# ketanfatania/QMRI-PnP-Recon-POC

Measured on NVIDIA B200. Metric: ADMM slice-iterations/s (224x224x10 slices; step = 120-slice PnP-ADMM recon + T1/T2/PD matching), higher is better.
Workload: dtype f32 (x-update fp32 FFT; denoiser split-bf16 tcgen05, fp32 accumulate; matching fp32)

## Files before the change

qmri-pnp-recon-poc_b200/csrc/conv_tc.cu:

```cuda
#include <cuda.h>
#include <cuda_bf16.h>
#include <math.h>
#include <stdlib.h>
#include <string.h>
#include <time.h>
#include <unistd.h>

#include "common.cuh"
#include "conv_kernels.h"

namespace {

constexpr int TC_THREADS = 192;
constexpr int PAIR_THREADS = 224;
constexpr int TC_BM = 128;
constexpr int TC_BK = 64;
constexpr uint32_t A_TILE_BYTES = TC_BM * TC_BK * 2;

template <int BN>
struct TcCfg {
    static constexpr uint32_t B_TILE_BYTES = BN * TC_BK * 2;
    static constexpr uint32_t STAGE_BYTES = 2 * A_TILE_BYTES + 2 * B_TILE_BYTES;
    static constexpr int STAGES = (BN == 64) ? 4 : 3;
    static constexpr uint32_t TMEM_COLS = 2 * BN;
// ... 76 lines not shown
        "elect.sync _|e, 0xffffffff;\n\t"
        "setp.ne.b32 p, %4, 0;\n\t"
        "@e tcgen05.mma.cta_group::1.kind::f16 [%0], %1, %2, %3, p;\n\t}"
        ::"r"(tmem_d), "l"(desc_a), "l"(desc_b), "r"(idesc), "r"(accumulate)
        : "memory");
}
__device__ __forceinline__ void tc_commit_elect(uint64_t* bar) {
    asm volatile(
        "{\n\t.reg .pred e;\n\t"
        "elect.sync _|e, 0xffffffff;\n\t"
        "@e tcgen05.commit.cta_group::1.mbarrier::arrive::one.shared::cluster.b64 [%0];\n\t}"
        ::"r"(smem_u32(bar))
        : "memory");
}

__device__ __forceinline__ uint64_t umma_desc(uint32_t saddr) {
    const uint64_t lo = (uint64_t)((saddr >> 4) & 0x3FFF) | ((uint64_t)1 << 16);
    const uint64_t hi = (uint64_t)64 | ((uint64_t)1 << 14) | ((uint64_t)2 << 29);
    return lo | (hi << 32);
}

__device__ __forceinline__ uint32_t pack_bf16(float a, float b) {
    __nv_bfloat162 t = __floats2bfloat162_rn(a, b);
    return *reinterpret_cast<uint32_t*>(&t);
}
__device__ __forceinline__ void unpack_bf16(uint32_t u, float& a, float& b) {
    a = __uint_as_float(u << 16);
    b = __uint_as_float(u & 0xffff0000u);
}


struct TcMaps {
    CUtensorMap a_hi[4], a_lo[4];
// ... 439 lines not shown
        __syncwarp();
        cluster_sync_all();
        if (warp >= 2) tc_epilogue_reduce_dsmem<BN>(p, reinterpret_cast<const float*>(smem), cs_row, (int)cluster_ctarank(), cs_o, cs_ok);
        __syncwarp();
        cluster_sync_all();
    }
    tc_fence_before();
    __syncthreads();
    if (warp == 1) {
        tc_fence_after();
        asm volatile("tcgen05.dealloc.cta_group::1.sync.aligned.b32 %0, %1;" ::"r"(tmem_base), "r"(Cfg::TMEM_COLS));
    }
}


template <int NA, int STACK>
struct PairCfg {
    static constexpr int NOUT = STACK ? NA / 2 : NA;
    static constexpr uint32_t A_PLANE = 20480;
    static constexpr uint32_t A_SLOT = 2 * A_PLANE;
    static constexpr uint32_t B1_BYTES = (NA / 2) * 128;
    static constexpr uint32_t B2_BYTES = STACK ? (NA / 4) * 128 : B1_BYTES;
    static constexpr uint32_t B_STAGE = B1_BYTES + B2_BYTES;
    static constexpr int AS = (NA == 128) ? 3 : 2;
    static constexpr int ASB = 4;
    static constexpr int BS = (NA == 128) ? 8 : (STACK ? 5 : 4);
    static constexpr bool DUAL_OK = STACK && NA == 128;
    static constexpr int EPW = DUAL_OK ? 8 : 4;
    static constexpr int THREADS = DUAL_OK ? 352 : PAIR_THREADS;
    static constexpr uint32_t TMEM_COLS = DUAL_OK ? 512 : 2 * NA;
    static constexpr uint32_t RESW_BYTES = 9 * B1_BYTES;
    static constexpr size_t STAGE_AREA = (size_t)AS * A_SLOT + (size_t)BS * B_STAGE;
    static constexpr size_t SMEM = STAGE_AREA + 1024 + 256;
};

__device__ __forceinline__ uint32_t mapa_rank(uint32_t saddr, uint32_t rank) {
    uint32_t r;
    asm volatile("mapa.shared::cluster.u32 %0, %1, %2;" : "=r"(r) : "r"(saddr), "r"(rank));
    return r;
}
__device__ __forceinline__ void mbar_arrive_cluster(uint32_t cluster_addr) {
    asm volatile("mbarrier.arrive.release.cluster.shared::cluster.b64 _, [%0];" ::"r"(cluster_addr) : "memory");
}
__device__ __forceinline__ void mbar_arrive_cluster_relaxed(uint32_t cluster_addr) {
    asm volatile("mbarrier.arrive.relaxed.cluster.shared::cluster.b64 _, [%0];" ::"r"(cluster_addr) : "memory");
}
__device__ __forceinline__ void tma2_load_4d(void* dst, const CUtensorMap* tm, uint32_t bar_cluster_addr, int c0, int c1, int c2, int c3) {
    asm volatile(
        "cp.async.bulk.tensor.4d.cta_group::2.shared::cluster.global.tile.mbarrier::complete_tx::bytes [%0], [%1, {%3, %4, %5, %6}], [%2];"
        ::"r"(smem_u32(dst)), "l"(tm), "r"(bar_cluster_addr), "r"(c0), "r"(c1), "r"(c2), "r"(c3)
        : "memory");
}
__device__ __forceinline__ void tma2_load_2d(void* dst, const CUtensorMap* tm, uint32_t bar_cluster_addr, int c0, int c1) {
    asm volatile(
        "cp.async.bulk.tensor.2d.cta_group::2.shared::cluster.global.tile.mbarrier::complete_tx::bytes [%0], [%1, {%3, %4}], [%2];"
        ::"r"(smem_u32(dst)), "l"(tm), "r"(bar_cluster_addr), "r"(c0), "r"(c1)
        : "memory");
}
__device__ __forceinline__ void tma_prefetch_l2_4d(const CUtensorMap* tm, int c0, int c1, int c2, int c3) {
    asm volatile("cp.async.bulk.prefetch.tensor.4d.L2.global.tile [%0, {%1, %2, %3, %4}];" ::"l"(tm), "r"(c0), "r"(c1), "r"(c2), "r"(c3) : "memory");
}
__device__ __forceinline__ void tc2_commit(uint64_t* bar) {
    asm volatile("tcgen05.commit.cta_group::2.mbarrier::arrive::one.shared::cluster.multicast::cluster.b64 [%0], %1;" ::"r"(smem_u32(bar)), "h"((uint16_t)3)
                 : "memory");
}
__device__ __forceinline__ void tc2_mma(uint32_t tmem_d, uint64_t desc_a, uint64_t desc_b, uint32_t idesc, uint32_t accumulate) {
    asm volatile(
        "{\n\t.reg .pred p;\n\t"
        "setp.ne.b32 p, %4, 0;\n\t"
        "tcgen05.mma.cta_group::2.kind::f16 [%0], %1, %2, %3, p;\n\t}"
        ::"r"(tmem_d), "l"(desc_a), "l"(desc_b), "r"(idesc), "r"(accumulate)
        : "memory");
}

__device__ __forceinline__ void tc2_mma_elect(uint32_t tmem_d, uint64_t desc_a, uint64_t desc_b, uint32_t idesc, uint32_t accumulate) {
    asm volatile(
        "{\n\t.reg .pred p, e;\n\t"
        "elect.sync _|e, 0xffffffff;\n\t"
        "setp.ne.b32 p, %4, 0;\n\t"
        "@e tcgen05.mma.cta_group::2.kind::f16 [%0], %1, %2, %3, p;\n\t}"
        ::"r"(tmem_d), "l"(desc_a), "l"(desc_b), "r"(idesc), "r"(accumulate)
        : "memory");
}
__device__ __forceinline__ void tc2_commit_elect(uint64_t* bar) {
    asm volatile(
        "{\n\t.reg .pred e;\n\t"
        "elect.sync _|e, 0xffffffff;\n\t"
        "@e tcgen05.commit.cta_group::2.mbarrier::arrive::one.shared::cluster.multicast::cluster.b64 [%0], %1;\n\t}"
        ::"r"(smem_u32(bar)), "h"((uint16_t)3)
        : "memory");
}

template <int NA, int STACK>
__device__ __forceinline__ void pair_acc16(uint32_t taddr, uint32_t taddr2, int c0, float* v, bool resw = false) {
    uint32_t a[16];
    tc_ld16(taddr + c0, a);
    if (STACK) {
        uint32_t b[16];
        tc_ld16(taddr + (resw ? (c0 < NA / 4 ? 3 * NA / 4 : NA / 4) : NA / 2) + c0, b);
        if (taddr2) {
            uint32_t c[16];
            tc_ld16(taddr2 + c0, c);
            tc_wait_ld();
#pragma unroll
            for (int j = 0; j < 16; ++j) v[j] = (__uint_as_float(a[j]) + __uint_as_float(c[j])) + __uint_as_float(b[j]);
        } else {
            tc_wait_ld();
#pragma unroll
            for (int j = 0; j < 16; ++j) v[j] = __uint_as_float(a[j]) + __uint_as_float(b[j]);
        }
    } else {
        tc_wait_ld();
#pragma unroll
        for (int j = 0; j < 16; ++j) v[j] = __uint_as_float(a[j]);
    }
}

template <int NA, int STACK>
__global__ void __launch_bounds__(PairCfg<NA, STACK>::THREADS, 1)
tc_conv3x3_pair_kernel(const __grid_constant__ CUtensorMap tmA_hi, const __grid_constant__ CUtensorMap tmA_lo,
                       const __grid_constant__ CUtensorMap tmB_hi, const __grid_constant__ CUtensorMap tmB_lo,
                       const __grid_constant__ CUtensorMap tmB_h2, const __grid_constant__ CUtensorMap tmB_l2,
                       const __grid_constant__ CUtensorMap tmO_hi, const __grid_constant__ CUtensorMap tmO_lo,
                       const __grid_constant__ CUtensorMap tmR_hi, const __grid_constant__ CUtensorMap tmR_lo, const TcK p) {
    using Cfg = PairCfg<NA, STACK>;
    constexpr int AS = Cfg::AS, BS = Cfg::BS, NOUT = Cfg::NOUT;
    extern __shared__ unsigned char tc_smem_raw[];
    const uint32_t raw = smem_u32(tc_smem_raw);
    unsigned char* smem = tc_smem_raw + ((1024u - (raw & 1023u)) & 1023u);
    unsigned char* smemB = smem + (size_t)AS * Cfg::A_SLOT;
    uint64_t* bars = reinterpret_cast<uint64_t*>(smemB + (size_t)BS * Cfg::B_STAGE);
    constexpr int ASB = Cfg::ASB;
    uint64_t* fullA = bars;
    uint64_t* emptyA = bars + ASB;
    uint64_t* fullB = bars + 2 * ASB;
    uint64_t* emptyB = bars + 2 * ASB + BS;
    uint64_t* tfull = bars + 2 * ASB + 2 * BS;
    uint64_t* tempty = tfull + 2;
    uint32_t* tmem_slot = reinterpret_cast<uint32_t*>(tempty + 2);

    const int warp = __shfl_sync(0xffffffffu, threadIdx.x >> 5, 0), lane = threadIdx.x & 31;
    const int cblocks = p.Cin / TC_BK;
    const int U = 3 * cblocks;
    const int NT = p.Cout / NOUT;
    const int tiles_xy = p.tiles_x * p.tiles_y;
    const int ptiles = tiles_xy * p.S;
    const int pgroups = (ptiles + 1) / 2;
    const int total_work = pgroups * NT * p.nsplit;
    const int crank = (int)cluster_ctarank();
    const int cidx = blockIdx.x >> 1, nclusters = gridDim.x >> 1;
    const uint32_t slab_bytes = (uint32_t)((p.BH + 2) * p.BW * 128);
    const uint32_t dy_bytes = (uint32_t)(p.BW * 128);
    const bool dual = Cfg::DUAL_OK && (p.dual & 1);
    const bool resw = Cfg::DUAL_OK && p.resw && p.Cin == TC_BK;
    const uint32_t a_stage = resw ? 2 * slab_bytes : Cfg::A_SLOT;
    const uint32_t a_plane = resw ? slab_bytes : Cfg::A_PLANE;
    const bool tma_out = resw && p.tma_out;
    const bool res_tma = tma_out && p.res_tma;
    constexpr uint32_t OUT_BYTES = 2 * TC_BM * 128;
    const int obufs = p.tma_out == 1 ? 1 : 2;
    const int as_fit = (int)((Cfg::STAGE_AREA - Cfg::RESW_BYTES - (tma_out ? obufs * OUT_BYTES : 0u)) / (2 * slab_bytes));
    uint64_t* fullR = fullB + 2;
    uint64_t* emptyR = fullB + 4;
    uint64_t* outFull = fullB + 6;
    const int as_cap = (p.resw >= 2 && p.resw < Cfg::ASB) ? p.resw : Cfg::ASB;
    const int AS_EFF = resw ? (as_fit < as_cap ? as_fit : as_cap) : AS;
    unsigned char* smemW = smem;
    unsigned char* smemO = smem + Cfg::RESW_BYTES;
    unsigned char* smemA = resw ? smem + Cfg::RESW_BYTES + (tma_out ? obufs * OUT_BYTES : 0u) : smem;

    if (threadIdx.x == 0) {
        const uint32_t nissue = dual ? 2u : 1u;
        for (int s = 0; s < ASB; ++s) {
            mbar_init(&fullA[s], 1);
            mbar_init(&emptyA[s], nissue);
        }
        for (int s = 0; s < BS; ++s) {
            mbar_init(&fullB[s], 1);
            mbar_init(&emptyB[s], nissue);
        }
        for (int a = 0; a < 2; ++a) {
            mbar_init(&tfull[a], nissue);
            mbar_init(&tempty[a], 2 * Cfg::EPW);
            if (tma_out) mbar_init(&outFull[a], Cfg::EPW);
        }
        asm volatile("fence.mbarrier_init.release.cluster;" ::: "memory");
        tma_prefetch_desc(&tmA_hi);
        tma_prefetch_desc(&tmA_lo);
        tma_prefetch_desc(&tmB_hi);
        tma_prefetch_desc(&tmB_lo);
        tma_prefetch_desc(&tmB_h2);
        tma_prefetch_desc(&tmB_l2);
        tma_prefetch_desc(&tmO_hi);
        tma_prefetch_desc(&tmO_lo);
        tma_prefetch_desc(&tmR_hi);
        tma_prefetch_desc(&tmR_lo);
    }
// ... 30 lines not shown
                const int r = w / p.nsplit;
                const int nt = r % NT;
                const int pt = (r / NT) * 2 + crank;
                const int txy = pt % tiles_xy;
                const int s = (pt < ptiles) ? pt / tiles_xy : p.S;
                const int x0 = (txy % p.tiles_x) * p.BW, y0 = (txy / p.tiles_x) * p.BH;
                const int u0 = (split * U) / p.nsplit, u1 = ((split + 1) * U) / p.nsplit;
                if (p.l2pf && w + nclusters < total_work) {
                    const int w2 = w + nclusters;
                    const int r2 = w2 / p.nsplit, split2 = w2 % p.nsplit;
                    const int pt2 = (r2 / NT) * 2 + crank;
                    if (pt2 < ptiles) {
                        const int txy2 = pt2 % tiles_xy, s2 = pt2 / tiles_xy;
                        const int px0 = (txy2 % p.tiles_x) * p.BW, py0 = (txy2 / p.tiles_x) * p.BH;
                        const int v0 = (split2 * U) / p.nsplit, v1 = ((split2 + 1) * U) / p.nsplit;
                        for (int u = v0; u < v1; ++u) {
                            const int cb = u / 3, dxi = u - 3 * cb;
                            tma_prefetch_l2_4d(&tmA_hi, cb * TC_BK, px0 + dxi - 1, py0 - 1, s2);
                            tma_prefetch_l2_4d(&tmA_lo, cb * TC_BK, px0 + dxi - 1, py0 - 1, s2);
                        }
                    }
                }
                for (int u = u0; u < u1; ++u) {
                    const int cb = u / 3, dxi = u - 3 * cb;
                    TC_TRACE(0, (w << 12) | (u << 4) | 1);
                    {
                        TC_PROF_T0();
                        mbar_wait(&emptyA[sa], pa ^ 1);
                        TC_PROF_ADD(prof_w5);
                    }
                    unsigned char* st = smemA + (size_t)sa * a_stage;
                    if (p.dual & 256) {
                        if (crank == 0) mbar_arrive(&fullA[sa]);
                    } else {
                    if (crank == 0) mbar_expect_tx(&fullA[sa], 4 * slab_bytes);
                    const uint32_t barA = mapa_rank(smem_u32(&fullA[sa]), 0);
                    tma2_load_4d(st, &tmA_hi, barA, cb * TC_BK, x0 + dxi - 1, y0 - 1, s);
                    tma2_load_4d(st + a_plane, &tmA_lo, barA, cb * TC_BK, x0 + dxi - 1, y0 - 1, s);
                    }
                    if (++sa == AS_EFF) {
                        sa = 0;
                        pa ^= 1;
                    }
                    for (int dyi = 0; dyi < 3 && !resw; ++dyi) {
                        const int kcol = (dyi * 3 + dxi) * p.Cin + cb * TC_BK;
                        TC_TRACE(0, (w << 12) | (u << 4) | (2 + dyi));
                        mbar_wait(&emptyB[sb], pb ^ 1);
                        unsigned char* sbp = smemB + (size_t)sb * Cfg::B_STAGE;
                        if (crank == 0) mbar_expect_tx(&fullB[sb], 2 * Cfg::B_STAGE);
                        const uint32_t barB = mapa_rank(smem_u32(&fullB[sb]), 0);
                        if (STACK) {
                            tma2_load_2d(sbp, crank == 0 ? &tmB_hi : &tmB_lo, barB, kcol, 0);
                            tma2_load_2d(sbp + Cfg::B1_BYTES, &tmB_h2, barB, kcol, crank * (NOUT / 2));
                        } else {
                            tma2_load_2d(sbp, &tmB_hi, barB, kcol, nt * NOUT + crank * (NA / 2));
                            tma2_load_2d(sbp + Cfg::B1_BYTES, &tmB_lo, barB, kcol, nt * NOUT + crank * (NA / 2));
                        }
// ... 25 lines not shown
            for (int w = cidx; w < total_work; w += nclusters, ++it) {
                const int split = w % p.nsplit;
                const int u0 = (split * U) / p.nsplit, u1 = ((split + 1) * U) / p.nsplit;
                const int ab = it & 1;
                const uint32_t aphase = (it >> 1) & 1;
                if (lane == 0) TC_TRACE(1, (w << 12) | 0xF00);
                {
                    TC_PROF_T0();
                    mbar_wait(&tempty[ab], aphase ^ 1);
                    TC_PROF_ADD(prof_w1);
                    ++prof_n;
                }
                tc_fence_after();
                const uint32_t tmem_d = tmem_base + (uint32_t)(ab * NA);
                for (int u = u0; u < u1; ++u) {
                    if (lane == 0) TC_TRACE(1, (w << 12) | (u << 4) | 1);
                    {
                        TC_PROF_T0();
                        mbar_wait(&fullA[sa], pa);
                        TC_PROF_ADD(prof_w0);
                    }
                    tc_fence_after();
                    const uint32_t ha = smem_u32(smemA + (size_t)sa * a_stage);
                    const long long issue_t0 = p.prof ? clock64() : 0;
                    for (int dyi = 0; dyi < 3; ++dyi) {
                        if (lane == 0) TC_TRACE(1, (w << 12) | (u << 4) | (2 + dyi));
                        if (!resw) {
                            mbar_wait(&fullB[sb], pb);
                            tc_fence_after();
                        }
                        if (p.dual & 16) continue;
                        const uint32_t sbase = resw ? smem_u32(smemW + (size_t)(dyi * 3 + (u - 3 * (u / 3))) * Cfg::B1_BYTES)
                                                    : smem_u32(smemB + (size_t)sb * Cfg::B_STAGE);
                        const uint64_t a_hi = umma_desc(ha + dyi * dy_bytes), a_lo = umma_desc(ha + a_plane + dyi * dy_bytes);
                        const uint64_t b_1 = umma_desc(sbase), b_2 = umma_desc(resw ? sbase : sbase + Cfg::B1_BYTES);
#pragma unroll
                        for (int k = 0; k < TC_BK / 16; ++k) {
                            const uint64_t ko = (uint64_t)(k * 2);
                            const uint32_t acc = ((u - u0) | dyi | k) ? 1u : 0u;
                            if (STACK) {
                                tc2_mma_elect(tmem_d, a_hi + ko, b_1 + ko, idesc_full, acc);
                                if (!dual) tc2_mma_elect(tmem_d, a_lo + ko, b_2 + ko, idesc_half, 1u);
                            } else {
                                tc2_mma_elect(tmem_d, a_hi + ko, b_1 + ko, idesc_full, acc);
                                tc2_mma_elect(tmem_d, a_hi + ko, b_2 + ko, idesc_full, 1u);
                                tc2_mma_elect(tmem_d, a_lo + ko, b_1 + ko, idesc_full, 1u);
                            }
                        }
                        if (!resw) {
                            tc2_commit_elect(&emptyB[sb]);
                            if (++sb == BS) {
                                sb = 0;
                                pb ^= 1;
                            }
                        }
                    }
                    if (p.prof) prof_w8 += (unsigned long long)(clock64() - issue_t0);
                    {
                        TC_PROF_T0();
                        tc2_commit_elect(&emptyA[sa]);
                        TC_PROF_ADD(prof_w9);
                    }
                    if (++sa == AS_EFF) {
                        sa = 0;
                        pa ^= 1;
                    }
                }
                {
                    TC_PROF_T0();
                    tc2_commit_elect(&tfull[ab]);
                    TC_PROF_ADD(prof_w9);
                }
            }
            if (lane == 0) {
            TC_PROF_PUT(8, prof_w8);
            TC_PROF_PUT(9, prof_w9);
            TC_PROF_PUT(2, clock64() - role_t0);
            }
            if (p.prof && lane == 0) {
                unsigned long long role_ns1;
// ... 25 lines not shown
                const int txy = pt % tiles_xy, s = pt / tiles_xy;
                const int sbuf = obufs == 2 ? (it & 1) : 0;
                mbar_wait(&outFull[sbuf], (uint32_t)(obufs == 2 ? it >> 1 : it) & 1u);
                if (pt < ptiles && !(p.dual & 32)) {
                    const int tx0 = (txy % p.tiles_x) * p.BW, ty0 = (txy / p.tiles_x) * p.BH;
                    tma_store_4d(&tmO_hi, smem_u32(smemO) + (uint32_t)sbuf * OUT_BYTES, 0, tx0, ty0, s);
                    tma_store_4d(&tmO_lo, smem_u32(smemO) + (uint32_t)sbuf * OUT_BYTES + TC_BM * 128u, 0, tx0, ty0, s);
                }
                asm volatile("cp.async.bulk.commit_group;" ::: "memory");
                asm volatile("cp.async.bulk.wait_group.read 0;" ::: "memory");
                if (res_tma) load_residual(w + obufs * nclusters, sbuf);
                else mbar_arrive(&emptyR[sbuf]);
            }
            asm volatile("cp.async.bulk.wait_group 0;" ::: "memory");
        }
        if (lane == 0 && crank == 0 && dual) {
            const uint32_t idesc_half = (1u << 4) | (1u << 7) | (1u << 10) | ((uint32_t)(256 >> 4) << 24) | ((uint32_t)((NA / 2) >> 3) << 17);
            int sa = 0, sb = 0;
            uint32_t pa = 0, pb = 0;
            int it = 0;
            for (int w = cidx; w < total_work; w += nclusters, ++it) {
                const int split = w % p.nsplit;
                const int u0 = (split * U) / p.nsplit, u1 = ((split + 1) * U) / p.nsplit;
                const int ab = it & 1;
                const uint32_t aphase = (it >> 1) & 1;
                if (resw && it == 0) {
                    mbar_wait(&fullB[0], 0);
                    tc_fence_after();
                }
                mbar_wait(&tempty[ab], aphase ^ 1);
                tc_fence_after();
                const uint32_t tmem_d2 = tmem_base + (uint32_t)(2 * NA + ab * (NA / 2));
                for (int u = u0; u < u1; ++u) {
                    mbar_wait(&fullA[sa], pa);
                    tc_fence_after();
                    const uint32_t ha = smem_u32(smemA + (size_t)sa * a_stage);
                    for (int dyi = 0; dyi < 3; ++dyi) {
                        if (!resw) {
                            mbar_wait(&fullB[sb], pb);
                            tc_fence_after();
                        }
                        const uint32_t sbase = resw ? smem_u32(smemW + (size_t)(dyi * 3 + (u - 3 * (u / 3))) * Cfg::B1_BYTES)
                                                    : smem_u32(smemB + (size_t)sb * Cfg::B_STAGE);
                        const uint64_t a_lo = umma_desc(ha + a_plane + dyi * dy_bytes);
                        const uint64_t b_2 = umma_desc(resw ? sbase : sbase + Cfg::B1_BYTES);
#pragma unroll
                        for (int k = 0; k < TC_BK / 16; ++k) {
                            const uint64_t ko = (uint64_t)(k * 2);
                            tc2_mma(tmem_d2, a_lo + ko, b_2 + ko, idesc_half, ((u - u0) | dyi | k) ? 1u : 0u);
                        }
                        if (!resw) {
                            tc2_commit(&emptyB[sb]);
                            if (++sb == BS) {
                                sb = 0;
                                pb ^= 1;
                            }
                        }
                    }
                    tc2_commit(&emptyA[sa]);
                    if (++sa == AS_EFF) {
                        sa = 0;
                        pa ^= 1;
                    }
                }
                tc2_commit(&tfull[ab]);
            }
        }
    } else {
        const int lg = warp & 3;
        const int row = lg * 32 + lane;
        int it = 0;
        const long long role_t0 = p.prof ? clock64() : 0;
        unsigned long long prof_w3 = 0, prof_w10 = 0, prof_w11 = 0, prof_w12 = 0, prof_w13 = 0;
        for (int w = cidx; w < total_work; w += nclusters, ++it) {
            const int split = w % p.nsplit;
            const int r = w / p.nsplit;
            const int ab = it & 1;
            const uint32_t aphase = (it >> 1) & 1;
            const int nt = r % NT;
            const int pt = (r / NT) * 2 + crank;
            const bool live = pt < ptiles;
            const int txy = pt % tiles_xy;
            const int s = pt / tiles_xy;
            const int x = (txy % p.tiles_x) * p.BW + row % p.BW;
            const int y = (txy / p.tiles_x) * p.BH + row / p.BW;
            const bool ok = live && (x < p.W) && (y < p.H);
            const size_t o = (((size_t)s * p.H + y) * p.W + x) * p.Cout + (size_t)nt * NOUT;
            const uint32_t taddr = tmem_base + ((uint32_t)(lg * 32) << 16) + (uint32_t)(ab * NA);
            const uint32_t taddr2 = dual ? tmem_base + ((uint32_t)(lg * 32) << 16) + (uint32_t)(2 * NA + ab * (NA / 2)) : 0u;
            const uint32_t tempty_leader = mapa_rank(smem_u32(&tempty[ab]), 0);
            if (lane == 0) TC_TRACE(2 + lg, (w << 12) | 1);
            if (p.nsplit == 1) {
                if constexpr (Cfg::DUAL_OK) {
                    const int sbuf = obufs == 2 ? (it & 1) : 0;
                    const uint32_t suse = (uint32_t)(obufs == 2 ? it >> 1 : it);
                    const uint32_t orow_hi = smem_u32(smemO) + (uint32_t)sbuf * OUT_BYTES + (uint32_t)row * 128u, orow_lo = orow_hi + TC_BM * 128u;
                    const int r7 = row & 7;
                    const bool g_r1 = ok && !res_tma && (p.res1_hi != nullptr), g_r2 = ok && (p.res2_hi != nullptr);
                    uint4 q2[4];
                    if (g_r2) {
                        const int c0 = (Cfg::EPW == 8 && warp >= 7) ? NOUT / 2 : 0;
                        q2[0] = *reinterpret_cast<const uint4*>(p.res2_hi + o + c0);
                        q2[1] = *reinterpret_cast<const uint4*>(p.res2_hi + o + c0 + 8);
                        q2[2] = *reinterpret_cast<const uint4*>(p.res2_lo + o + c0);
                        q2[3] = *reinterpret_cast<const uint4*>(p.res2_lo + o + c0 + 8);
                    }
                    if (tma_out) {
                        TC_PROF_T0();
                        if (res_tma) mbar_wait(&fullR[sbuf], suse & 1u);
                        else mbar_wait(&emptyR[sbuf], (suse & 1u) ^ 1u);
// ... 93 lines not shown
                            const uint4* gl = reinterpret_cast<const uint4*>(p.res2_lo + o + h0);
    #pragma unroll
                            for (int i = 0; i < PRE / 8; ++i) add_split8(rs + 8 * i, gh[i], gl[i]);
                        }
                        if (h0 == 0) {
                            TC_PROF_T0();
                            mbar_wait(&tfull[ab], aphase);
                            TC_PROF_ADD(prof_w3);
                            tc_fence_after();
                        }
                        if (p.dual & 32) continue;
    #pragma unroll
                        for (int c1 = 0; c1 < PRE; c1 += 16) {
                            const int cc = h0 + c1;
                            float v[16];
                            pair_acc16<NA, STACK>(taddr, taddr2, cc, v, resw);
                            if (has_r1 || has_r2) {
    #pragma unroll
                                for (int j = 0; j < 16; ++j) v[j] += rs[c1 + j];
                            }
                            if (ok) store_split16(p.out_hi + o + cc, p.out_lo + o + cc, v, p.relu);
                        }
                    }
                    tc_fence_before();
                    __syncwarp();
                    if (lane == 0) mbar_arrive_cluster(tempty_leader);
                }
            } else {
                mbar_wait(&tfull[ab], aphase);
                tc_fence_after();
                const int t = pt * NT + nt;
                float* prow0 = p.partial + ((size_t)t * p.nsplit * TC_BM + row) * NOUT;
                if (live) {
                    float* prow = prow0 + (size_t)split * TC_BM * NOUT;
#pragma unroll 1
                    for (int cc = 0; cc < NOUT; cc += 16) {
                        float v[16];
                        pair_acc16<NA, STACK>(taddr, taddr2, cc, v, resw);
                        float4* d = reinterpret_cast<float4*>(prow + cc);
#pragma unroll
                        for (int q = 0; q < 4; ++q) d[q] = make_float4(v[4 * q], v[4 * q + 1], v[4 * q + 2], v[4 * q + 3]);
                    }
                }
                tc_fence_before();
                __syncwarp();
                if (lane == 0) mbar_arrive_cluster(tempty_leader);
                if (live) {
                    __threadfence();
                    __syncwarp();
                    int old = 0;
                    if (lane == 0) old = atomicAdd(&p.tickets[t * 4 + lg], 1);
                    old = __shfl_sync(0xffffffffu, old, 0);
                    if (old == p.nsplit - 1) {
                        __threadfence();
                        if (lane == 0) p.tickets[t * 4 + lg] = 0;
                        if (ok) tc_epilogue_reduce<NOUT>(p, prow0, o);
                    }
                }
            }
        }
        if (threadIdx.x == 64) {
            TC_PROF_PUT(4, clock64() - role_t0);
            TC_PROF_PUT(3, prof_w3);
            TC_PROF_PUT(10, prof_w10);
            TC_PROF_PUT(11, prof_w11);
            TC_PROF_PUT(12, prof_w12);
            TC_PROF_PUT(13, prof_w13);
        }
    }
    if (lane == 0) TC_TRACE(6, 0x1000 + warp);
    tc_fence_before();
    __syncthreads();
    if (threadIdx.x == 0) TC_TRACE(7, 1);
    cluster_sync_all();
    if (warp == 1) {
        tc_fence_after();
        asm volatile("tcgen05.dealloc.cta_group::2.sync.aligned.b32 %0, %1;" ::"r"(tmem_base), "r"(Cfg::TMEM_COLS));
// ... 208 lines not shown
    k.tma_out = 0;
    k.res_tma = 0;
    k.l2pf = 0;
    k.prof = nullptr;
    if (BN == 64) {
        if (p.mode == TC_CONV3X3) return launch_tc<64, 0>(ctx, maps, k, grid);
        if (p.mode == TC_DOWN2X2) return launch_tc<64, 1>(ctx, maps, k, grid);
        return launch_tc<64, 2>(ctx, maps, k, grid);
    }
    if (p.mode == TC_CONV3X3) return launch_tc<128, 0>(ctx, maps, k, grid);
    if (p.mode == TC_DOWN2X2) return launch_tc<128, 1>(ctx, maps, k, grid);
    return launch_tc<128, 2>(ctx, maps, k, grid);
}

int tc_slab_tile_shape(int W, int H, int* BW, int* BH) {
    const int cand[2][2] = {{16, 8}, {8, 16}};
    int best = 0;
    double best_eff = -1;
    for (int i = 0; i < 2; ++i) {
        int bw = cand[i][0], bh = cand[i][1];
        double eff = ((double)W * H) / ((double)((W + bw - 1) / bw * bw) * ((H + bh - 1) / bh * bh));
        if (i == 1) eff *= 1.04;
        if (eff > best_eff + 1e-9) {
            best_eff = eff;
            best = i;
        }
    }
    *BW = cand[best][0];
    *BH = cand[best][1];
    return QMRI_OK;
}

void tc_pair_weight_boxes(int Cout, int* rows_main, int* rows_h2) {
    if (Cout >= 256) {
        *rows_main = 128;
        *rows_h2 = 128;
    } else {
        *rows_main = Cout;
        *rows_h2 = Cout / 2;
    }
}

template <int NA, int STACK>
static int launch_pair(qmri_ctx* ctx, const TcConvParams& p, TcK k) {
// ... 11 lines not shown
    const int U = 3 * (p.Cin / TC_BK);
    int nsplit = 1;
    if (p.partial && p.tickets && 2 * groups <= max_clusters) {
        nsplit = max_clusters / groups;
        if (nsplit > U / 2) nsplit = U / 2;
        if (nsplit > 8) nsplit = 8;
        if (nsplit < 1) nsplit = 1;
    }
    k.nsplit = nsplit;
    const int work = groups * nsplit;
    const int nclusters = work < max_clusters ? work : max_clusters;
    cudaLaunchConfig_t cfg = {};
    static const int dual_on = getenv("QMRI_TC_DUAL") ? atoi(getenv("QMRI_TC_DUAL")) : 0;
    static const bool resw_off = getenv("QMRI_TC_RESW") && !strcmp(getenv("QMRI_TC_RESW"), "0");
    static const int resw_stages = getenv("QMRI_TC_RESW") ? atoi(getenv("QMRI_TC_RESW")) : 1;
    k.dual = Cfg::DUAL_OK ? (dual_on & ~1) : 0;
    static const int dbg_layer = getenv("QMRI_TC_DBG_LAYER") ? atoi(getenv("QMRI_TC_DBG_LAYER")) : -1;
    static int launch_no = 0;
    bool dbg_this = true;
    if (Cfg::DUAL_OK && dbg_layer >= 0) {
        dbg_this = (launch_no++ % 16) == dbg_layer;
        if (!dbg_this) k.dual = 0;
    }
    k.resw = (Cfg::DUAL_OK && !resw_off && p.Cin == TC_BK) ? (resw_stages >= 2 ? resw_stages : 1) : 0;
    const char* tmaout_s = getenv("QMRI_TC_TMAOUT");
    const bool tma_out_off = tmaout_s && !strcmp(tmaout_s, "0");
    const char* outbuf_s = getenv("QMRI_TC_OUTBUF");
    const int outbuf_env = outbuf_s ? atoi(outbuf_s) : 0;
    k.tma_out = (k.resw && p.mapO_hi && p.mapO_lo && !tma_out_off) ? (outbuf_env == 1 || outbuf_env == 2 ? outbuf_env : (p.res1_hi ? 2 : 1)) : 0;
    k.res_tma = (k.tma_out && p.res1_hi && p.mapR_hi && p.mapR_lo) ? 1 : 0;
    static const int l2pf_env = getenv("QMRI_TC_L2PF") ? atoi(getenv("QMRI_TC_L2PF")) : 0;
    k.l2pf = l2pf_env > 0 ? 1 : 0;
    cfg.gridDim = dim3(nclusters * 2);
    cfg.blockDim = dim3(Cfg::THREADS);
    cfg.dynamicSmemBytes = Cfg::SMEM;
    cfg.stream = ctx->stream;
    cudaLaunchAttribute attr[2];
    attr[0].id = cudaLaunchAttributeClusterDimension;
    attr[0].val.clusterDim.x = 2;
    attr[0].val.clusterDim.y = 1;
    attr[0].val.clusterDim.z = 1;
    attr[1].id = cudaLaunchAttributeProgrammaticStreamSerialization;
    attr[1].val.programmaticStreamSerializationAllowed = tc_pdl_enabled() ? 1 : 0;
    cfg.attrs = attr;
// ... 298 lines not shown
    cfg.dynamicSmemBytes = SW_SMEM;
    cfg.stream = ctx->stream;
    cudaLaunchAttribute attr[1];
    attr[0].id = cudaLaunchAttributeProgrammaticStreamSerialization;
    attr[0].val.programmaticStreamSerializationAllowed = tc_pdl_enabled() ? 1 : 0;
    cfg.attrs = attr;
    cfg.numAttrs = 1;
    QCUDA(cudaLaunchKernelEx(&cfg, tc_conv64_swap_kernel, *(const CUtensorMap*)p.mapA_hi[0], *(const CUtensorMap*)p.mapA_lo[0], (const SwapK)k));
    QLAUNCH_CHECK(ctx);
    return QMRI_OK;
}

int conv3x3_tc_pair(qmri_ctx* ctx, const TcConvParams& p) {
    if (p.Cin % TC_BK) return qmri_fail(QMRI_EINVAL, "conv3x3_tc_pair: Cin %% 64");
    if (p.Cout != 64 && p.Cout != 128 && p.Cout % 256) return qmri_fail(QMRI_EINVAL, "conv3x3_tc_pair: Cout %d", p.Cout);
    if (p.BW % 8 || p.BW * p.BH != TC_BM || (p.BH + 2) * p.BW * 128 > (int)PairCfg<256, 0>::A_PLANE)
        return qmri_fail(QMRI_EINVAL, "conv3x3_tc_pair: tile %d x %d not supported", p.BW, p.BH);
    if (!p.mapA_hi[0] || !p.mapA_lo[0] || !p.mapB_hi || !p.mapB_lo || !p.mapB_h2) return qmri_fail(QMRI_EINVAL, "conv3x3_tc_pair: missing tensor map");
    TcK k;
    k.out_hi = p.out_hi; k.out_lo = p.out_lo;
    k.res1_hi = p.res1_hi; k.res1_lo = p.res1_lo;
    k.res2_hi = p.res2_hi; k.res2_lo = p.res2_lo;
    k.partial = p.partial; k.tickets = p.tickets;
    k.S = p.S; k.H = p.H; k.W = p.W; k.Cin = p.Cin; k.Cout = p.Cout;
    k.BW = p.BW; k.BH = p.BH; k.tiles_x = p.tiles_x; k.tiles_y = p.tiles_y;
    k.relu = p.relu; k.nsplit = 1; k.trace = nullptr; k.cluster_splitk = 0; k.dual = 0; k.resw = 0; k.tma_out = 0; k.res_tma = 0; k.l2pf = 0; k.prof = nullptr;
    if (p.Cout == 64) return launch_pair<128, 1>(ctx, p, k);
    if (p.Cout == 128) return launch_pair<256, 1>(ctx, p, k);
    return launch_pair<256, 0>(ctx, p, k);
}
```

qmri-pnp-recon-poc_b200/csrc/unetres.cu:

```cuda
#include <stdlib.h>
#include <string.h>

#include <vector>

#include "common.cuh"
#include "conv_kernels.h"
#include "unetres.h"

static const int NC[4] = {64, 128, 256, 512};

namespace {

struct LayerDesc {
    int kind;
    int cin, cout;
};

std::vector<LayerDesc> layer_table(int in_nc) {
    std::vector<LayerDesc> L;
    L.push_back({3, in_nc, NC[0]});
    for (int lvl = 0; lvl < 3; ++lvl) {
        for (int i = 0; i < 8; ++i) L.push_back({0, NC[lvl], NC[lvl]});
        L.push_back({1, NC[lvl], NC[lvl + 1]});
    }
// ... 295 lines not shown
    }
}

static int build_act_maps(qmri_net* net, int H, int W) {
    if (net->amap_ws == net->ws && net->amap_chunk == net->chunk && net->amap_H == H && net->amap_W == W) return QMRI_OK;
    uint16_t *hi[3][4], *lo[3][4];
    tc_buffers(net, H, W, hi, lo);
    for (int l = 0; l < 4; ++l) {
        int BW, BH;
        tc_tile_shape(W >> l, H >> l, &BW, &BH);
        for (int b = 0; b < 3; ++b) {
            QCHECK(tc_make_act_map(&net->amap[b][l][0], hi[b][l], net->chunk, H >> l, W >> l, NC[l], BW, BH));
            QCHECK(tc_make_act_map(&net->amap[b][l][1], lo[b][l], net->chunk, H >> l, W >> l, NC[l], BW, BH));
            int SW, SH;
            tc_slab_tile_shape(W >> l, H >> l, &SW, &SH);
            QCHECK(tc_make_act_map(&net->amap_slab[b][l][0], hi[b][l], net->chunk, H >> l, W >> l, NC[l], SW, SH + 2));
            QCHECK(tc_make_act_map(&net->amap_slab[b][l][1], lo[b][l], net->chunk, H >> l, W >> l, NC[l], SW, SH + 2));
            if (l == 0) {
                QCHECK(tc_make_act_map(&net->amap_tile[b][0], hi[b][0], net->chunk, H, W, NC[0], SW, SH));
                QCHECK(tc_make_act_map(&net->amap_tile[b][1], lo[b][0], net->chunk, H, W, NC[0], SW, SH));
            }
            if (l == 0 && conv64_swap_supported(W, H, NC[0], NC[0])) {
                QCHECK(tc_make_act_map(&net->amap_swap[b][0], hi[b][0], net->chunk, H, W, NC[0], 16, 16));
                QCHECK(tc_make_act_map(&net->amap_swap[b][1], lo[b][0], net->chunk, H, W, NC[0], 16, 16));
            }
            if (l < 3) {
                int DW, DH;
                tc_tile_shape(W >> (l + 1), H >> (l + 1), &DW, &DH);
                for (int tap = 0; tap < 4; ++tap) {
                    QCHECK(tc_make_down_map(&net->amap_down[b][l][tap][0], hi[b][l], net->chunk, H >> l, W >> l, NC[l], tap >> 1, tap & 1, DW, DH));
                    QCHECK(tc_make_down_map(&net->amap_down[b][l][tap][1], lo[b][l], net->chunk, H >> l, W >> l, NC[l], tap >> 1, tap & 1, DW, DH));
                }
// ... 241 lines not shown
```

Before: 1664.

## Load one halo slab per channel block and reuse it across dx taps

The pair conv kernel now TMA-loads a single (BW+2)x(BH+2) halo slab per 64-channel block, instead of three dx-shifted slabs. The MMA descriptors offset into it by dxi*128 bytes with a row stride of (BW+2)*128. This cuts A-operand TMA traffic and mbarrier round-trips per channel block roughly threefold, with the slab tile fixed at 8x16. The experimental dual-issue MMA path is removed, and the L2 prefetch is simplified to one prefetch per channel block. The fixed tile shape may pad worse for some layer sizes, and the non-default descriptor stride must match the swizzled layout.

```diff
diff --git a/qmri-pnp-recon-poc_b200/csrc/conv_tc.cu b/qmri-pnp-recon-poc_b200/csrc/conv_tc.cu
--- a/qmri-pnp-recon-poc_b200/csrc/conv_tc.cu
+++ b/qmri-pnp-recon-poc_b200/csrc/conv_tc.cu
@@ -114,9 +114,9 @@
         : "memory");
 }
 
-__device__ __forceinline__ uint64_t umma_desc(uint32_t saddr) {
+__device__ __forceinline__ uint64_t umma_desc(uint32_t saddr, uint32_t sbo = 1024) {
     const uint64_t lo = (uint64_t)((saddr >> 4) & 0x3FFF) | ((uint64_t)1 << 16);
-    const uint64_t hi = (uint64_t)64 | ((uint64_t)1 << 14) | ((uint64_t)2 << 29);
+    const uint64_t hi = (uint64_t)(sbo >> 4) | ((uint64_t)1 << 14) | ((uint64_t)2 << 29);
     return lo | (hi << 32);
 }
 
@@ -586,24 +586,30 @@
 }
 
 
+constexpr int PAIR_BW = 8, PAIR_BH = 16;
 template <int NA, int STACK>
 struct PairCfg {
     static constexpr int NOUT = STACK ? NA / 2 : NA;
-    static constexpr uint32_t A_PLANE = 20480;
+    static constexpr uint32_t SLAB_BYTES = (PAIR_BW + 2) * (PAIR_BH + 2) * 128;
+    static constexpr uint32_t A_PLANE = (SLAB_BYTES + 1023) & ~1023u;
     static constexpr uint32_t A_SLOT = 2 * A_PLANE;
     static constexpr uint32_t B1_BYTES = (NA / 2) * 128;
     static constexpr uint32_t B2_BYTES = STACK ? (NA / 4) * 128 : B1_BYTES;
     static constexpr uint32_t B_STAGE = B1_BYTES + B2_BYTES;
-    static constexpr int AS = (NA == 128) ? 3 : 2;
+    static constexpr int AS = 2;
     static constexpr int ASB = 4;
     static constexpr int BS = (NA == 128) ? 8 : (STACK ? 5 : 4);
-    static constexpr bool DUAL_OK = STACK && NA == 128;
-    static constexpr int EPW = DUAL_OK ? 8 : 4;
-    static constexpr int THREADS = DUAL_OK ? 352 : PAIR_THREADS;
-    static constexpr uint32_t TMEM_COLS = DUAL_OK ? 512 : 2 * NA;
+    static constexpr bool C64 = STACK && NA == 128;
+    static constexpr int EPW = C64 ? 8 : 4;
+    static constexpr int THREADS = C64 ? 352 : PAIR_THREADS;
+    static constexpr uint32_t TMEM_COLS = 2 * NA;
     static constexpr uint32_t RESW_BYTES = 9 * B1_BYTES;
-    static constexpr size_t STAGE_AREA = (size_t)AS * A_SLOT + (size_t)BS * B_STAGE;
+    static constexpr uint32_t OUT_BYTES = 2 * TC_BM * 128;
+    static constexpr size_t RESW_AREA = (size_t)RESW_BYTES + OUT_BYTES + 2 * (size_t)A_SLOT;
+    static constexpr size_t RING_AREA = (size_t)AS * A_SLOT + (size_t)BS * B_STAGE;
+    static constexpr size_t STAGE_AREA = (C64 && RESW_AREA > RING_AREA) ? RESW_AREA : RING_AREA;
     static constexpr size_t SMEM = STAGE_AREA + 1024 + 256;
+    static_assert(SMEM <= 227 * 1024, "pair kernel: dynamic shared memory over 227 KB");
 };
 
 __device__ __forceinline__ uint32_t mapa_rank(uint32_t saddr, uint32_t rank) {
@@ -631,18 +637,6 @@
 }
 __device__ __forceinline__ void tma_prefetch_l2_4d(const CUtensorMap* tm, int c0, int c1, int c2, int c3) {
     asm volatile("cp.async.bulk.prefetch.tensor.4d.L2.global.tile [%0, {%1, %2, %3, %4}];" ::"l"(tm), "r"(c0), "r"(c1), "r"(c2), "r"(c3) : "memory");
-}
-__device__ __forceinline__ void tc2_commit(uint64_t* bar) {
-    asm volatile("tcgen05.commit.cta_group::2.mbarrier::arrive::one.shared::cluster.multicast::cluster.b64 [%0], %1;" ::"r"(smem_u32(bar)), "h"((uint16_t)3)
-                 : "memory");
-}
-__device__ __forceinline__ void tc2_mma(uint32_t tmem_d, uint64_t desc_a, uint64_t desc_b, uint32_t idesc, uint32_t accumulate) {
-    asm volatile(
-        "{\n\t.reg .pred p;\n\t"
-        "setp.ne.b32 p, %4, 0;\n\t"
-        "tcgen05.mma.cta_group::2.kind::f16 [%0], %1, %2, %3, p;\n\t}"
-        ::"r"(tmem_d), "l"(desc_a), "l"(desc_b), "r"(idesc), "r"(accumulate)
-        : "memory");
 }
 
 __device__ __forceinline__ void tc2_mma_elect(uint32_t tmem_d, uint64_t desc_a, uint64_t desc_b, uint32_t idesc, uint32_t accumulate) {
@@ -664,23 +658,15 @@
 }
 
 template <int NA, int STACK>
-__device__ __forceinline__ void pair_acc16(uint32_t taddr, uint32_t taddr2, int c0, float* v, bool resw = false) {
+__device__ __forceinline__ void pair_acc16(uint32_t taddr, int c0, float* v, bool resw = false) {
     uint32_t a[16];
     tc_ld16(taddr + c0, a);
     if (STACK) {
         uint32_t b[16];
         tc_ld16(taddr + (resw ? (c0 < NA / 4 ? 3 * NA / 4 : NA / 4) : NA / 2) + c0, b);
-        if (taddr2) {
-            uint32_t c[16];
-            tc_ld16(taddr2 + c0, c);
-            tc_wait_ld();
-#pragma unroll
-            for (int j = 0; j < 16; ++j) v[j] = (__uint_as_float(a[j]) + __uint_as_float(c[j])) + __uint_as_float(b[j]);
-        } else {
-            tc_wait_ld();
-#pragma unroll
-            for (int j = 0; j < 16; ++j) v[j] = __uint_as_float(a[j]) + __uint_as_float(b[j]);
-        }
+        tc_wait_ld();
+#pragma unroll
+        for (int j = 0; j < 16; ++j) v[j] = __uint_as_float(a[j]) + __uint_as_float(b[j]);
     } else {
         tc_wait_ld();
 #pragma unroll
@@ -701,7 +687,7 @@
     const uint32_t raw = smem_u32(tc_smem_raw);
     unsigned char* smem = tc_smem_raw + ((1024u - (raw & 1023u)) & 1023u);
     unsigned char* smemB = smem + (size_t)AS * Cfg::A_SLOT;
-    uint64_t* bars = reinterpret_cast<uint64_t*>(smemB + (size_t)BS * Cfg::B_STAGE);
+    uint64_t* bars = reinterpret_cast<uint64_t*>(smem + Cfg::STAGE_AREA);
     constexpr int ASB = Cfg::ASB;
     uint64_t* fullA = bars;
     uint64_t* emptyA = bars + ASB;
@@ -721,17 +707,12 @@
     const int total_work = pgroups * NT * p.nsplit;
     const int crank = (int)cluster_ctarank();
     const int cidx = blockIdx.x >> 1, nclusters = gridDim.x >> 1;
-    const uint32_t slab_bytes = (uint32_t)((p.BH + 2) * p.BW * 128);
-    const uint32_t dy_bytes = (uint32_t)(p.BW * 128);
-    const bool dual = Cfg::DUAL_OK && (p.dual & 1);
-    const bool resw = Cfg::DUAL_OK && p.resw && p.Cin == TC_BK;
-    const uint32_t a_stage = resw ? 2 * slab_bytes : Cfg::A_SLOT;
-    const uint32_t a_plane = resw ? slab_bytes : Cfg::A_PLANE;
+    const bool resw = Cfg::C64 && p.resw && p.Cin == TC_BK;
     const bool tma_out = resw && p.tma_out;
     const bool res_tma = tma_out && p.res_tma;
-    constexpr uint32_t OUT_BYTES = 2 * TC_BM * 128;
-    const int obufs = p.tma_out == 1 ? 1 : 2;
-    const int as_fit = (int)((Cfg::STAGE_AREA - Cfg::RESW_BYTES - (tma_out ? obufs * OUT_BYTES : 0u)) / (2 * slab_bytes));
+    constexpr uint32_t OUT_BYTES = Cfg::OUT_BYTES;
+    const int obufs = p.tma_out == 2 ? 2 : 1;
+    const int as_fit = (int)((Cfg::STAGE_AREA - Cfg::RESW_BYTES - (tma_out ? obufs * OUT_BYTES : 0u)) / Cfg::A_SLOT);
     uint64_t* fullR = fullB + 2;
     uint64_t* emptyR = fullB + 4;
     uint64_t* outFull = fullB + 6;
@@ -742,17 +723,16 @@
     unsigned char* smemA = resw ? smem + Cfg::RESW_BYTES + (tma_out ? obufs * OUT_BYTES : 0u) : smem;
 
     if (threadIdx.x == 0) {
-        const uint32_t nissue = dual ? 2u : 1u;
         for (int s = 0; s < ASB; ++s) {
             mbar_init(&fullA[s], 1);
-            mbar_init(&emptyA[s], nissue);
+            mbar_init(&emptyA[s], 1);
         }
         for (int s = 0; s < BS; ++s) {
             mbar_init(&fullB[s], 1);
-            mbar_init(&emptyB[s], nissue);
+            mbar_init(&emptyB[s], 1);
         }
         for (int a = 0; a < 2; ++a) {
-            mbar_init(&tfull[a], nissue);
+            mbar_init(&tfull[a], 1);
             mbar_init(&tempty[a], 2 * Cfg::EPW);
             if (tma_out) mbar_init(&outFull[a], Cfg::EPW);
         }
@@ -813,33 +793,34 @@
                         const int txy2 = pt2 % tiles_xy, s2 = pt2 / tiles_xy;
                         const int px0 = (txy2 % p.tiles_x) * p.BW, py0 = (txy2 / p.tiles_x) * p.BH;
                         const int v0 = (split2 * U) / p.nsplit, v1 = ((split2 + 1) * U) / p.nsplit;
-                        for (int u = v0; u < v1; ++u) {
-                            const int cb = u / 3, dxi = u - 3 * cb;
-                            tma_prefetch_l2_4d(&tmA_hi, cb * TC_BK, px0 + dxi - 1, py0 - 1, s2);
-                            tma_prefetch_l2_4d(&tmA_lo, cb * TC_BK, px0 + dxi - 1, py0 - 1, s2);
+                        for (int cb = v0 / 3; cb <= (v1 - 1) / 3; ++cb) {
+                            tma_prefetch_l2_4d(&tmA_hi, cb * TC_BK, px0 - 1, py0 - 1, s2);
+                            tma_prefetch_l2_4d(&tmA_lo, cb * TC_BK, px0 - 1, py0 - 1, s2);
                         }
                     }
                 }
                 for (int u = u0; u < u1; ++u) {
                     const int cb = u / 3, dxi = u - 3 * cb;
                     TC_TRACE(0, (w << 12) | (u << 4) | 1);
-                    {
-                        TC_PROF_T0();
-                        mbar_wait(&emptyA[sa], pa ^ 1);
-                        TC_PROF_ADD(prof_w5);
-                    }
-                    unsigned char* st = smemA + (size_t)sa * a_stage;
-                    if (p.dual & 256) {
-                        if (crank == 0) mbar_arrive(&fullA[sa]);
-                    } else {
-                    if (crank == 0) mbar_expect_tx(&fullA[sa], 4 * slab_bytes);
-                    const uint32_t barA = mapa_rank(smem_u32(&fullA[sa]), 0);
-                    tma2_load_4d(st, &tmA_hi, barA, cb * TC_BK, x0 + dxi - 1, y0 - 1, s);
-                    tma2_load_4d(st + a_plane, &tmA_lo, barA, cb * TC_BK, x0 + dxi - 1, y0 - 1, s);
-                    }
-                    if (++sa == AS_EFF) {
-                        sa = 0;
-                        pa ^= 1;
+                    if (u == u0 || dxi == 0) {
+                        {
+                            TC_PROF_T0();
+                            mbar_wait(&emptyA[sa], pa ^ 1);
+                            TC_PROF_ADD(prof_w5);
+                        }
+                        unsigned char* st = smemA + (size_t)sa * Cfg::A_SLOT;
+                        if (p.dual & 256) {
+                            if (crank == 0) mbar_arrive(&fullA[sa]);
+                        } else {
+                            if (crank == 0) mbar_expect_tx(&fullA[sa], 4 * Cfg::SLAB_BYTES);
+                            const uint32_t barA = mapa_rank(smem_u32(&fullA[sa]), 0);
+                            tma2_load_4d(st, &tmA_hi, barA, cb * TC_BK, x0 - 1, y0 - 1, s);
+                            tma2_load_4d(st + Cfg::A_PLANE, &tmA_lo, barA, cb * TC_BK, x0 - 1, y0 - 1, s);
+                        }
+                        if (++sa == AS_EFF) {
+                            sa = 0;
+                            pa ^= 1;
+                        }
                     }
                     for (int dyi = 0; dyi < 3 && !resw; ++dyi) {
                         const int kcol = (dyi * 3 + dxi) * p.Cin + cb * TC_BK;
@@ -895,14 +876,15 @@
                 tc_fence_after();
                 const uint32_t tmem_d = tmem_base + (uint32_t)(ab * NA);
                 for (int u = u0; u < u1; ++u) {
+                    const int dxi = u - 3 * (u / 3);
                     if (lane == 0) TC_TRACE(1, (w << 12) | (u << 4) | 1);
-                    {
+                    if (u == u0 || dxi == 0) {
                         TC_PROF_T0();
                         mbar_wait(&fullA[sa], pa);
                         TC_PROF_ADD(prof_w0);
-                    }
-                    tc_fence_after();
-                    const uint32_t ha = smem_u32(smemA + (size_t)sa * a_stage);
+                        tc_fence_after();
+                    }
+                    const uint32_t ha = smem_u32(smemA + (size_t)sa * Cfg::A_SLOT) + (uint32_t)dxi * 128u;
                     const long long issue_t0 = p.prof ? clock64() : 0;
                     for (int dyi = 0; dyi < 3; ++dyi) {
                         if (lane == 0) TC_TRACE(1, (w << 12) | (u << 4) | (2 + dyi));
@@ -911,9 +893,10 @@
                             tc_fence_after();
                         }
                         if (p.dual & 16) continue;
-                        const uint32_t sbase = resw ? smem_u32(smemW + (size_t)(dyi * 3 + (u - 3 * (u / 3))) * Cfg::B1_BYTES)
+                        const uint32_t sbase = resw ? smem_u32(smemW + (size_t)(dyi * 3 + dxi) * Cfg::B1_BYTES)
                                                     : smem_u32(smemB + (size_t)sb * Cfg::B_STAGE);
-                        const uint64_t a_hi = umma_desc(ha + dyi * dy_bytes), a_lo = umma_desc(ha + a_plane + dyi * dy_bytes);
+                        constexpr uint32_t SROW = (PAIR_BW + 2) * 128;
+                        const uint64_t a_hi = umma_desc(ha + dyi * SROW, SROW), a_lo = umma_desc(ha + Cfg::A_PLANE + dyi * SROW, SROW);
                         const uint64_t b_1 = umma_desc(sbase), b_2 = umma_desc(resw ? sbase : sbase + Cfg::B1_BYTES);
 #pragma unroll
                         for (int k = 0; k < TC_BK / 16; ++k) {
@@ -921,7 +904,7 @@
                             const uint32_t acc = ((u - u0) | dyi | k) ? 1u : 0u;
                             if (STACK) {
                                 tc2_mma_elect(tmem_d, a_hi + ko, b_1 + ko, idesc_full, acc);
-                                if (!dual) tc2_mma_elect(tmem_d, a_lo + ko, b_2 + ko, idesc_half, 1u);
+                                tc2_mma_elect(tmem_d, a_lo + ko, b_2 + ko, idesc_half, 1u);
                             } else {
                                 tc2_mma_elect(tmem_d, a_hi + ko, b_1 + ko, idesc_full, acc);
                                 tc2_mma_elect(tmem_d, a_hi + ko, b_2 + ko, idesc_full, 1u);
@@ -937,14 +920,14 @@
                         }
                     }
                     if (p.prof) prof_w8 += (unsigned long long)(clock64() - issue_t0);
-                    {
+                    if (dxi == 2 || u == u1 - 1) {
                         TC_PROF_T0();
                         tc2_commit_elect(&emptyA[sa]);
                         TC_PROF_ADD(prof_w9);
-                    }
-                    if (++sa == AS_EFF) {
-                        sa = 0;
-                        pa ^= 1;
+                        if (++sa == AS_EFF) {
+                            sa = 0;
+                            pa ^= 1;
+                        }
                     }
                 }
                 {
@@ -1000,63 +983,11 @@
             }
             asm volatile("cp.async.bulk.wait_group 0;" ::: "memory");
         }
-        if (lane == 0 && crank == 0 && dual) {
-            const uint32_t idesc_half = (1u << 4) | (1u << 7) | (1u << 10) | ((uint32_t)(256 >> 4) << 24) | ((uint32_t)((NA / 2) >> 3) << 17);
-            int sa = 0, sb = 0;
-            uint32_t pa = 0, pb = 0;
-            int it = 0;
-            for (int w = cidx; w < total_work; w += nclusters, ++it) {
-                const int split = w % p.nsplit;
-                const int u0 = (split * U) / p.nsplit, u1 = ((split + 1) * U) / p.nsplit;
-                const int ab = it & 1;
-                const uint32_t aphase = (it >> 1) & 1;
-                if (resw && it == 0) {
-                    mbar_wait(&fullB[0], 0);
-                    tc_fence_after();
-                }
-                mbar_wait(&tempty[ab], aphase ^ 1);
-                tc_fence_after();
-                const uint32_t tmem_d2 = tmem_base + (uint32_t)(2 * NA + ab * (NA / 2));
-                for (int u = u0; u < u1; ++u) {
-                    mbar_wait(&fullA[sa], pa);
-                    tc_fence_after();
-                    const uint32_t ha = smem_u32(smemA + (size_t)sa * a_stage);
-                    for (int dyi = 0; dyi < 3; ++dyi) {
-                        if (!resw) {
-                            mbar_wait(&fullB[sb], pb);
-                            tc_fence_after();
-                        }
-                        const uint32_t sbase = resw ? smem_u32(smemW + (size_t)(dyi * 3 + (u - 3 * (u / 3))) * Cfg::B1_BYTES)
-                                                    : smem_u32(smemB + (size_t)sb * Cfg::B_STAGE);
-                        const uint64_t a_lo = umma_desc(ha + a_plane + dyi * dy_bytes);
-                        const uint64_t b_2 = umma_desc(resw ? sbase : sbase + Cfg::B1_BYTES);
-#pragma unroll
-                        for (int k = 0; k < TC_BK / 16; ++k) {
-                            const uint64_t ko = (uint64_t)(k * 2);
-                            tc2_mma(tmem_d2, a_lo + ko, b_2 + ko, idesc_half, ((u - u0) | dyi | k) ? 1u : 0u);
-                        }
-                        if (!resw) {
-                            tc2_commit(&emptyB[sb]);
-                            if (++sb == BS) {
-                                sb = 0;
-                                pb ^= 1;
-                            }
-                        }
-                    }
-                    tc2_commit(&emptyA[sa]);
-                    if (++sa == AS_EFF) {
-                        sa = 0;
-                        pa ^= 1;
-                    }
-                }
-                tc2_commit(&tfull[ab]);
-            }
-        }
     } else {
         const int lg = warp & 3;
         const int row = lg * 32 + lane;
         int it = 0;
-        const long long role_t0 = p.prof ? clock64() : 0;
+        if (threadIdx.x == 64) TC_PROF_PUT(4, clock64());
         unsigned long long prof_w3 = 0, prof_w10 = 0, prof_w11 = 0, prof_w12 = 0, prof_w13 = 0;
         for (int w = cidx; w < total_work; w += nclusters, ++it) {
             const int split = w % p.nsplit;
@@ -1073,13 +1004,12 @@
             const bool ok = live && (x < p.W) && (y < p.H);
             const size_t o = (((size_t)s * p.H + y) * p.W + x) * p.Cout + (size_t)nt * NOUT;
             const uint32_t taddr = tmem_base + ((uint32_t)(lg * 32) << 16) + (uint32_t)(ab * NA);
-            const uint32_t taddr2 = dual ? tmem_base + ((uint32_t)(lg * 32) << 16) + (uint32_t)(2 * NA + ab * (NA / 2)) : 0u;
             const uint32_t tempty_leader = mapa_rank(smem_u32(&tempty[ab]), 0);
             if (lane == 0) TC_TRACE(2 + lg, (w << 12) | 1);
             if (p.nsplit == 1) {
-                if constexpr (Cfg::DUAL_OK) {
-                    const int sbuf = obufs == 2 ? (it & 1) : 0;
-                    const uint32_t suse = (uint32_t)(obufs == 2 ? it >> 1 : it);
+                if constexpr (Cfg::C64) {
+                    const int sbuf = p.tma_out == 2 ? (it & 1) : 0;
+                    const uint32_t suse = (uint32_t)(p.tma_out == 2 ? it >> 1 : it);
                     const uint32_t orow_hi = smem_u32(smemO) + (uint32_t)sbuf * OUT_BYTES + (uint32_t)row * 128u, orow_lo = orow_hi + TC_BM * 128u;
                     const int r7 = row & 7;
                     const bool g_r1 = ok && !res_tma && (p.res1_hi != nullptr), g_r2 = ok && (p.res2_hi != nullptr);
@@ -1203,7 +1133,7 @@
                         for (int c1 = 0; c1 < PRE; c1 += 16) {
                             const int cc = h0 + c1;
                             float v[16];
-                            pair_acc16<NA, STACK>(taddr, taddr2, cc, v, resw);
+                            pair_acc16<NA, STACK>(taddr, cc, v, resw);
                             if (has_r1 || has_r2) {
     #pragma unroll
                                 for (int j = 0; j < 16; ++j) v[j] += rs[c1 + j];
@@ -1225,7 +1155,7 @@
 #pragma unroll 1
                     for (int cc = 0; cc < NOUT; cc += 16) {
                         float v[16];
-                        pair_acc16<NA, STACK>(taddr, taddr2, cc, v, resw);
+                        pair_acc16<NA, STACK>(taddr, cc, v, resw);
                         float4* d = reinterpret_cast<float4*>(prow + cc);
 #pragma unroll
                         for (int q = 0; q < 4; ++q) d[q] = make_float4(v[4 * q], v[4 * q + 1], v[4 * q + 2], v[4 * q + 3]);
@@ -1249,7 +1179,7 @@
             }
         }
         if (threadIdx.x == 64) {
-            TC_PROF_PUT(4, clock64() - role_t0);
+            if (p.prof) TC_PROF_PUT(4, clock64() - (long long)p.prof[blockIdx.x * 16 + 4]);
             TC_PROF_PUT(3, prof_w3);
             TC_PROF_PUT(10, prof_w10);
             TC_PROF_PUT(11, prof_w11);
@@ -1488,20 +1418,10 @@
 }
 
 int tc_slab_tile_shape(int W, int H, int* BW, int* BH) {
-    const int cand[2][2] = {{16, 8}, {8, 16}};
-    int best = 0;
-    double best_eff = -1;
-    for (int i = 0; i < 2; ++i) {
-        int bw = cand[i][0], bh = cand[i][1];
-        double eff = ((double)W * H) / ((double)((W + bw - 1) / bw * bw) * ((H + bh - 1) / bh * bh));
-        if (i == 1) eff *= 1.04;
-        if (eff > best_eff + 1e-9) {
-            best_eff = eff;
-            best = i;
-        }
-    }
-    *BW = cand[best][0];
-    *BH = cand[best][1];
+    (void)W;
+    (void)H;
+    *BW = PAIR_BW;
+    *BH = PAIR_BH;
     return QMRI_OK;
 }
 
@@ -1543,20 +1463,20 @@
     static const int dual_on = getenv("QMRI_TC_DUAL") ? atoi(getenv("QMRI_TC_DUAL")) : 0;
     static const bool resw_off = getenv("QMRI_TC_RESW") && !strcmp(getenv("QMRI_TC_RESW"), "0");
     static const int resw_stages = getenv("QMRI_TC_RESW") ? atoi(getenv("QMRI_TC_RESW")) : 1;
-    k.dual = Cfg::DUAL_OK ? (dual_on & ~1) : 0;
+    k.dual = Cfg::C64 ? (dual_on & ~1) : 0;
     static const int dbg_layer = getenv("QMRI_TC_DBG_LAYER") ? atoi(getenv("QMRI_TC_DBG_LAYER")) : -1;
     static int launch_no = 0;
     bool dbg_this = true;
-    if (Cfg::DUAL_OK && dbg_layer >= 0) {
+    if (Cfg::C64 && dbg_layer >= 0) {
         dbg_this = (launch_no++ % 16) == dbg_layer;
         if (!dbg_this) k.dual = 0;
     }
-    k.resw = (Cfg::DUAL_OK && !resw_off && p.Cin == TC_BK) ? (resw_stages >= 2 ? resw_stages : 1) : 0;
+    k.resw = (Cfg::C64 && !resw_off && p.Cin == TC_BK) ? (resw_stages >= 2 ? resw_stages : 1) : 0;
     const char* tmaout_s = getenv("QMRI_TC_TMAOUT");
     const bool tma_out_off = tmaout_s && !strcmp(tmaout_s, "0");
     const char* outbuf_s = getenv("QMRI_TC_OUTBUF");
     const int outbuf_env = outbuf_s ? atoi(outbuf_s) : 0;
-    k.tma_out = (k.resw && p.mapO_hi && p.mapO_lo && !tma_out_off) ? (outbuf_env == 1 || outbuf_env == 2 ? outbuf_env : (p.res1_hi ? 2 : 1)) : 0;
+    k.tma_out = (k.resw && p.mapO_hi && p.mapO_lo && !tma_out_off) ? (outbuf_env == 2 ? 2 : 1) : 0;
     k.res_tma = (k.tma_out && p.res1_hi && p.mapR_hi && p.mapR_lo) ? 1 : 0;
     static const int l2pf_env = getenv("QMRI_TC_L2PF") ? atoi(getenv("QMRI_TC_L2PF")) : 0;
     k.l2pf = l2pf_env > 0 ? 1 : 0;
@@ -1885,7 +1805,7 @@
 int conv3x3_tc_pair(qmri_ctx* ctx, const TcConvParams& p) {
     if (p.Cin % TC_BK) return qmri_fail(QMRI_EINVAL, "conv3x3_tc_pair: Cin %% 64");
     if (p.Cout != 64 && p.Cout != 128 && p.Cout % 256) return qmri_fail(QMRI_EINVAL, "conv3x3_tc_pair: Cout %d", p.Cout);
-    if (p.BW % 8 || p.BW * p.BH != TC_BM || (p.BH + 2) * p.BW * 128 > (int)PairCfg<256, 0>::A_PLANE)
+    if (p.BW != PAIR_BW || p.BH != PAIR_BH)
         return qmri_fail(QMRI_EINVAL, "conv3x3_tc_pair: tile %d x %d not supported", p.BW, p.BH);
     if (!p.mapA_hi[0] || !p.mapA_lo[0] || !p.mapB_hi || !p.mapB_lo || !p.mapB_h2) return qmri_fail(QMRI_EINVAL, "conv3x3_tc_pair: missing tensor map");
     TcK k;
diff --git a/qmri-pnp-recon-poc_b200/csrc/unetres.cu b/qmri-pnp-recon-poc_b200/csrc/unetres.cu
--- a/qmri-pnp-recon-poc_b200/csrc/unetres.cu
+++ b/qmri-pnp-recon-poc_b200/csrc/unetres.cu
@@ -333,8 +333,8 @@
             QCHECK(tc_make_act_map(&net->amap[b][l][1], lo[b][l], net->chunk, H >> l, W >> l, NC[l], BW, BH));
             int SW, SH;
             tc_slab_tile_shape(W >> l, H >> l, &SW, &SH);
-            QCHECK(tc_make_act_map(&net->amap_slab[b][l][0], hi[b][l], net->chunk, H >> l, W >> l, NC[l], SW, SH + 2));
-            QCHECK(tc_make_act_map(&net->amap_slab[b][l][1], lo[b][l], net->chunk, H >> l, W >> l, NC[l], SW, SH + 2));
+            QCHECK(tc_make_act_map(&net->amap_slab[b][l][0], hi[b][l], net->chunk, H >> l, W >> l, NC[l], SW + 2, SH + 2));
+            QCHECK(tc_make_act_map(&net->amap_slab[b][l][1], lo[b][l], net->chunk, H >> l, W >> l, NC[l], SW + 2, SH + 2));
             if (l == 0) {
                 QCHECK(tc_make_act_map(&net->amap_tile[b][0], hi[b][0], net->chunk, H, W, NC[0], SW, SH));
                 QCHECK(tc_make_act_map(&net->amap_tile[b][1], lo[b][0], net->chunk, H, W, NC[0], SW, SH));
```

New measurement: 1715, median of 6. 3.0% higher.
